# nyu-systems/Grendel-GS

Measured on AMD Instinct MI355X. Metric: training iters/sec (fwd+bwd), higher is better.
Workload: dtype f32

## Files before the change

### grendel-gs_amd/csrc/loss.hip

```cpp
#include "common.h"

namespace {

__constant__ const float WIN[11] = {1.0283801239e-03f, 7.5987582095e-03f, 3.6000773311e-02f, 1.0936068743e-01f,
                                    2.1300552785e-01f, 2.6601171494e-01f, 2.1300552785e-01f, 1.0936068743e-01f,
                                    3.6000773311e-02f, 7.5987582095e-03f, 1.0283801239e-03f};
constexpr int LT = 512;
constexpr int VO = 1024 / LT;
constexpr int TW = 32, TH = 32;
constexpr int HW = TW + 10, HH = TH + 10;
constexpr int HSTR = TW + 8;
constexpr int TS = TW;
constexpr float SSIM_C1 = 0.01f * 0.01f;
constexpr float SSIM_C2 = 0.03f * 0.03f;

__device__ __forceinline__ float block_sum(float v, float *smem) {
    const int lane = threadIdx.x & 63, wave = threadIdx.x >> 6;
#pragma unroll
    for (int d = 32; d >= 1; d >>= 1) v += __shfl_xor(v, d, 64);
    if (lane == 0) smem[wave] = v;
    __syncthreads();
    float r = 0.f;
    for (int w = 0; w < LT / 64; w++) r += smem[w];
    __syncthreads();
    return r;
}

typedef float v2f __attribute__((ext_vector_type(2)));

__device__ __forceinline__ int loss_tile(int gxT, int gyT, int &c, int &ox, int &oy, int nwg) {
    const int lin = gsr_xcd_span_of_block(blockIdx.x, nwg);
    c = lin / (gxT * gyT);
    const int rem = lin - c * (gxT * gyT);
    const int by = rem / gxT;
    ox = (rem - by * gxT) * TW;
    oy = by * TH;
    return lin;
}
__device__ __forceinline__ bool loss_band(const int *__restrict__ band, int rows_cap, int W, int gxT, int &rows, int &gyT,
                                          int &nwg, long long &row_off) {
    nwg = gridDim.x;
    row_off = 0;
    if (!band) return true;
    const int channels = nwg / (gxT * gyT);
    const int y0 = band[0], y1 = band[1];
    rows = max(0, min(y1 - y0, rows_cap));
    gyT = (rows + TH - 1) / TH;
    nwg = channels * gxT * gyT;
    row_off = (long long)y0 * W;
    return (int)blockIdx.x < nwg;
}
constexpr int HV = (TW + 16) / 4;
static_assert(HH * HV <= LT, "one halo vector per thread");

__device__ __forceinline__ float expo_apply(const float *e, float x0, float x1, float x2) {
    return fmaf(e[0], x0, fmaf(e[1], x1, fmaf(e[2], x2, e[3])));
}

template <bool VEC, bool EXPO>
__global__ void __launch_bounds__(LT)
l1_ssim_forward_kernel(int rows, int W, int gxT, int gyT, const float *__restrict__ image, long long img_cstride,
                       const uint8_t *__restrict__ gt, float *__restrict__ partials, float *__restrict__ M1,
                       float *__restrict__ M2, float *__restrict__ M3, const int *__restrict__ band,
                       const float *__restrict__ expo) {
    __shared__ v2f sXY[HH][HW + 1];
    __shared__ v2f hAB[HH][HSTR];
    __shared__ v2f hCD[HH][HSTR];
    __shared__ float hE[HH][HSTR];
    __shared__ float red[LT / 64];
#ifndef GSR_ABL_LOSS_TWO_REDUCTIONS
    __shared__ float red2[LT / 64];
#endif
    int c, ox, oy, nwg;
    long long row_off;
    const int rows_cap = rows;
    if (!loss_band(band, rows_cap, W, gxT, rows, gyT, nwg, row_off)) {
        if (threadIdx.x < 2) partials[2 * (size_t)blockIdx.x + threadIdx.x] = 0.f;
        return;
    }
    const int tile_id = loss_tile(gxT, gyT, c, ox, oy, nwg);
    const int tid = threadIdx.x;
    const float *img_c = image + (long long)c * img_cstride + row_off;
    const uint8_t *gt_c = gt + (size_t)c * rows_cap * W;
    float e[4] = {0.f, 0.f, 0.f, 0.f};
    if (EXPO) {
#pragma unroll
        for (int i = 0; i < 4; i++) e[i] = expo[4 * c + i];
    }
    const float *img_0 = image + row_off;
    if (VEC) {
        if (tid < HH * HV) {
            const int ly = tid / HV, q = tid - ly * HV;
            const int gy = oy + ly - 5, gx0 = ox - 8 + 4 * q;
            float4 x = make_float4(0.f, 0.f, 0.f, 0.f);
            uchar4 y = make_uchar4(0, 0, 0, 0);
            if (gy >= 0 && gy < rows && gx0 >= 0 && gx0 < W) {
                if (EXPO) {
                    const float *p = img_0 + (size_t)gy * W + gx0;
                    const float4 x0 = *reinterpret_cast<const float4 *>(p);
                    const float4 x1 = *reinterpret_cast<const float4 *>(p + img_cstride);
                    const float4 x2 = *reinterpret_cast<const float4 *>(p + 2 * img_cstride);
                    x = make_float4(expo_apply(e, x0.x, x1.x, x2.x), expo_apply(e, x0.y, x1.y, x2.y),
                                    expo_apply(e, x0.z, x1.z, x2.z), expo_apply(e, x0.w, x1.w, x2.w));
                } else {
                    x = *reinterpret_cast<const float4 *>(img_c + (size_t)gy * W + gx0);
                }
                y = *reinterpret_cast<const uchar4 *>(gt_c + (size_t)gy * W + gx0);
            }
            const float xs[4] = {x.x, x.y, x.z, x.w};
            const float ys[4] = {(float)y.x, (float)y.y, (float)y.z, (float)y.w};
#pragma unroll
            for (int i = 0; i < 4; i++) {
                const int lx = 4 * q - 3 + i;
                if (lx >= 0 && lx < HW) sXY[ly][lx] = v2f{xs[i], ys[i] * (1.0f / 255.0f)};
            }
        }
    } else {
        for (int idx = tid; idx < HH * HW; idx += LT) {
            const int ly = idx / HW, lx = idx % HW;
            const int gy = oy + ly - 5, gx = ox + lx - 5;
            v2f v = {0.f, 0.f};
            if (gy >= 0 && gy < rows && gx >= 0 && gx < W) {
                if (EXPO) {
                    const float *p = img_0 + (size_t)gy * W + gx;
                    v.x = expo_apply(e, p[0], p[img_cstride], p[2 * img_cstride]);
                } else {
                    v.x = img_c[(size_t)gy * W + gx];
                }
                v.y = (float)gt_c[(size_t)gy * W + gx] * (1.0f / 255.0f);
            }
            sXY[ly][lx] = v;
        }
    }
    __syncthreads();
    for (int task = tid; task < HH * (TW / 4); task += LT) {
        const int r = task / (TW / 4), cx0 = (task % (TW / 4)) * 4;
        v2f xy[14], sq[14];
        float pr[14];
#pragma unroll
        for (int i = 0; i < 14; i++) {
            xy[i] = sXY[r][cx0 + i];
            sq[i] = xy[i] * xy[i];
            pr[i] = xy[i].x * xy[i].y;
#ifndef GSR_ABL_LOSS_FWD_OUTPUT_PAIRS
            asm("" : "+v"(pr[i]));
#endif
        }
#pragma unroll
        for (int o = 0; o < 4; o++) {
            v2f a = {0.f, 0.f}, b = {0.f, 0.f};
            float e = 0.f;
#pragma unroll
            for (int k = 0; k < 11; k++) {
                const float w = WIN[k];
                a += xy[o + k] * w;
                b += sq[o + k] * w;
                e += pr[o + k] * w;
            }
            hAB[r][cx0 + o] = a;
            hCD[r][cx0 + o] = b;
            hE[r][cx0 + o] = e;
        }
    }
    __syncthreads();
    const int tx = tid % TW, ty0 = (tid / TW) * VO;
    v2f vab[VO], vcd[VO];
    float ve[VO];
    {
        v2f p[10 + VO], q[10 + VO];
        float t[10 + VO];
#pragma unroll
        for (int i = 0; i < 10 + VO; i++) {
            p[i] = hAB[ty0 + i][tx];
            q[i] = hCD[ty0 + i][tx];
            t[i] = hE[ty0 + i][tx];
#ifndef GSR_ABL_LOSS_FWD_OUTPUT_PAIRS
            asm("" : "+v"(t[i]));
#endif
        }
#pragma unroll
        for (int o = 0; o < VO; o++) {
            v2f a = {0.f, 0.f}, b = {0.f, 0.f};
            float e = 0.f;
#pragma unroll
            for (int k = 0; k < 11; k++) {
                const float w = WIN[k];
                a += p[o + k] * w;
                b += q[o + k] * w;
                e += t[o + k] * w;
            }
            vab[o] = a;
            vcd[o] = b;
            ve[o] = e;
        }
    }
    const int gx = ox + tx;
    float l1 = 0.f, ssim_sum = 0.f;
#pragma unroll
    for (int o = 0; o < VO; o++) {
        const int ty = ty0 + o, gy = oy + ty;
        if (gy < rows && gx < W) {
            const float mu1 = vab[o].x, mu2 = vab[o].y, e11 = vcd[o].x, e22 = vcd[o].y, e12 = ve[o];
            const v2f cxy = sXY[ty + 5][tx + 5];
            const float x = cxy.x, y = cxy.y;
            const float mu1_sq = mu1 * mu1, mu2_sq = mu2 * mu2, mu12 = mu1 * mu2;
            const float s1 = e11 - mu1_sq, s2 = e22 - mu2_sq, s12 = e12 - mu12;
            const float A = 2.f * mu12 + SSIM_C1, B = 2.f * s12 + SSIM_C2;
            const float Cd = mu1_sq + mu2_sq + SSIM_C1, Dd = s1 + s2 + SSIM_C2;
            const float inv_d = __builtin_amdgcn_rcpf(Dd);
            const float inv = __builtin_amdgcn_rcpf(Cd) * inv_d;
            const float ssim = A * B * inv;
            ssim_sum += ssim;
            l1 += fabsf(x - y);
            if (M1) {
                const size_t off = ((size_t)c * rows_cap + gy) * W + gx;
                M1[off] = 2.f * mu2 * (B - A) * inv - ssim * 2.f * mu1 * (Dd - Cd) * inv;
                M2[off] = -ssim * inv_d;
                M3[off] = 2.f * A * inv;
            }
        }
    }
#ifdef GSR_ABL_LOSS_TWO_REDUCTIONS
    const float sl1 = block_sum(l1, red);
    const float sss = block_sum(ssim_sum, red);
#else
    float sl1 = l1, sss = ssim_sum;
#pragma unroll
    for (int d = 32; d >= 1; d >>= 1) sl1 += __shfl_xor(sl1, d, 64);
#pragma unroll
    for (int d = 32; d >= 1; d >>= 1) sss += __shfl_xor(sss, d, 64);
    if ((tid & 63) == 0) {
        red[tid >> 6] = sl1;
        red2[tid >> 6] = sss;
    }
    __syncthreads();
    sl1 = sss = 0.f;
    for (int w = 0; w < LT / 64; w++) sl1 += red[w];
    for (int w = 0; w < LT / 64; w++) sss += red2[w];
#endif
    if (tid == 0) {
        partials[2 * (size_t)tile_id] = sl1;
        partials[2 * (size_t)tile_id + 1] = sss;
    }
}

template <bool VEC>
__global__ void __launch_bounds__(LT)
l1_ssim_backward_kernel(int rows, int W, int gxT, int gyT, const float *__restrict__ image, long long img_cstride,
                        const uint8_t *__restrict__ gt, const float *__restrict__ M1, const float *__restrict__ M2,
                        const float *__restrict__ M3, const float *__restrict__ grad_l1_sum,
                        const float *__restrict__ grad_ssim_sum, float scale_l1, float scale_ssim,
                        float *__restrict__ grad_image, long long grad_cstride, const int *__restrict__ band) {
    __shared__ float sM[3][HH][HW + 1];
    __shared__ float hor[3][HH][HSTR];
    int c, ox, oy, nwg;
    long long row_off;
    const int rows_cap = rows;
    if (!loss_band(band, rows_cap, W, gxT, rows, gyT, nwg, row_off)) return;
    loss_tile(gxT, gyT, c, ox, oy, nwg);
    const int tid = threadIdx.x;
    const size_t cbase = (size_t)c * rows_cap * W;
    if (VEC) {
        if (tid < HH * HV) {
            const int ly = tid / HV, q = tid - ly * HV;
            const int gy = oy + ly - 5, gx0 = ox - 8 + 4 * q;
            float4 a = make_float4(0.f, 0.f, 0.f, 0.f), b = a, d = a;
            if (gy >= 0 && gy < rows && gx0 >= 0 && gx0 < W) {
                const size_t o = cbase + (size_t)gy * W + gx0;
                a = *reinterpret_cast<const float4 *>(M1 + o);
                b = *reinterpret_cast<const float4 *>(M2 + o);
                d = *reinterpret_cast<const float4 *>(M3 + o);
            }
            const float as[4] = {a.x, a.y, a.z, a.w}, bs[4] = {b.x, b.y, b.z, b.w}, ds[4] = {d.x, d.y, d.z, d.w};
#pragma unroll
            for (int i = 0; i < 4; i++) {
                const int lx = 4 * q - 3 + i;
                if (lx >= 0 && lx < HW) {
                    sM[0][ly][lx] = as[i];
                    sM[1][ly][lx] = bs[i];
                    sM[2][ly][lx] = ds[i];
                }
            }
        }
    } else {
        for (int idx = tid; idx < HH * HW; idx += LT) {
            const int ly = idx / HW, lx = idx % HW;
            const int gy = oy + ly - 5, gx = ox + lx - 5;
            float a = 0.f, b = 0.f, d = 0.f;
            if (gy >= 0 && gy < rows && gx >= 0 && gx < W) {
                const size_t o = cbase + (size_t)gy * W + gx;
                a = M1[o];
                b = M2[o];
                d = M3[o];
            }
            sM[0][ly][lx] = a;
            sM[1][ly][lx] = b;
            sM[2][ly][lx] = d;
        }
    }
    __syncthreads();
    for (int task = tid; task < HH * (TW / 4); task += LT) {
        const int r = task / (TW / 4), cx0 = (task % (TW / 4)) * 4;
#pragma unroll
        for (int m = 0; m < 3; m++) {
            float v[14];
#pragma unroll
            for (int i = 0; i < 14; i++) v[i] = sM[m][r][cx0 + i];
#pragma unroll
            for (int o = 0; o < 4; o++) {
                float a = 0.f;
#pragma unroll
                for (int k = 0; k < 11; k++) a += WIN[k] * v[o + k];
                hor[m][r][cx0 + o] = a;
            }
        }
    }
    __syncthreads();
    const int tx = tid % TW, ty0 = (tid / TW) * VO;
    float cv[3][VO];
#pragma unroll
    for (int m = 0; m < 3; m++) {
        float v[10 + VO];
#pragma unroll
        for (int i = 0; i < 10 + VO; i++) v[i] = hor[m][ty0 + i][tx];
#pragma unroll
        for (int o = 0; o < VO; o++) {
            float a = 0.f;
#pragma unroll
            for (int k = 0; k < 11; k++) a += WIN[k] * v[o + k];
            cv[m][o] = a;
        }
    }
    const int gx = ox + tx;
    if (gx >= W) return;
    const float gl1 = grad_l1_sum[0] * scale_l1, gss = grad_ssim_sum[0] * scale_ssim;
#pragma unroll
    for (int o = 0; o < VO; o++) {
        const int gy = oy + ty0 + o;
        if (gy >= rows) break;
        const float x = image[(long long)c * img_cstride + row_off + (size_t)gy * W + gx];
        const float y = (float)gt[cbase + (size_t)gy * W + gx] * (1.0f / 255.0f);
        const float d = x - y;
        const float sgn = (d > 0.f ? 1.f : 0.f) - (d < 0.f ? 1.f : 0.f);
        grad_image[(long long)c * grad_cstride + row_off + (size_t)gy * W + gx] =
            gl1 * sgn + gss * (cv[0][o] + 2.f * x * cv[1][o] + y * cv[2][o]);
    }
}

__global__ void __launch_bounds__(256) l1_ssim_finalize_kernel(int nb, const float *__restrict__ partials, float c_l1,
                                                                float c_ssim, float bias, float inv_n,
                                                                float *__restrict__ out) {
    __shared__ double red[2][4];
    double a = 0.0, b = 0.0;
    const float2 *p2 = reinterpret_cast<const float2 *>(partials);
    for (int i0 = threadIdx.x; i0 < nb; i0 += 256 * 8) {
        float2 v[8];
#pragma unroll
        for (int u = 0; u < 8; u++) v[u] = p2[min(i0 + 256 * u, nb - 1)];
#pragma unroll
        for (int u = 0; u < 8; u++)
            if (i0 + 256 * u < nb) {
                a += (double)v[u].x;
                b += (double)v[u].y;
            }
    }
#pragma unroll
    for (int d = 32; d >= 1; d >>= 1) {
        a += __shfl_xor(a, d, 64);
        b += __shfl_xor(b, d, 64);
    }
    if ((threadIdx.x & 63) == 0) {
        red[0][threadIdx.x >> 6] = a;
        red[1][threadIdx.x >> 6] = b;
    }
    __syncthreads();
    if (threadIdx.x == 0) {
        const float s1 = (float)(red[0][0] + red[0][1] + red[0][2] + red[0][3]);
        const float s2 = (float)(red[1][0] + red[1][1] + red[1][2] + red[1][3]);
        out[0] = c_l1 * s1 + c_ssim * s2 + bias;
        out[1] = s1 * inv_n;
        out[2] = s2 * inv_n;
    }
}

template <bool VEC>
__global__ void __launch_bounds__(LT)
l1_ssim_backward_exposure_kernel(int rows, int W, int gxT, int gyT, const float *__restrict__ image, long long img_cstride,
                                 const uint8_t *__restrict__ gt, const float *__restrict__ M1,
                                 const float *__restrict__ M2, const float *__restrict__ M3,
                                 const float *__restrict__ grad_l1_sum, const float *__restrict__ grad_ssim_sum,
                                 float scale_l1, float scale_ssim, float *__restrict__ grad_image, long long grad_cstride,
                                 const int *__restrict__ band, const float *__restrict__ expo,
                                 float *__restrict__ expo_partials) {
    __shared__ float sM[3][HH][HW + 1];
    __shared__ float hor[3][HH][HSTR];
    __shared__ float red[12][LT / 64];
    int c0, ox, oy, nwg;
    long long row_off;
    const int rows_cap = rows;
    if (!loss_band(band, rows_cap, W, gxT, rows, gyT, nwg, row_off)) {
        if (threadIdx.x < 12) expo_partials[12 * (size_t)blockIdx.x + threadIdx.x] = 0.f;
        return;
    }
    const int tile_id = loss_tile(gxT, gyT, c0, ox, oy, nwg);
    const int tid = threadIdx.x, lane = tid & 63, wave = tid >> 6;
    const int tx = tid % TW, ty0 = (tid / TW) * VO;
    const int gx = ox + tx;
    const float gl1 = grad_l1_sum[0] * scale_l1, gss = grad_ssim_sum[0] * scale_ssim;
    float xin[3][VO], gout[3][VO];
    bool ok[VO];
#pragma unroll
    for (int o = 0; o < VO; o++) {
        const int gy = oy + ty0 + o;
        ok[o] = gx < W && gy < rows;
#pragma unroll
        for (int k = 0; k < 3; k++) {
            xin[k][o] = ok[o] ? image[(long long)k * img_cstride + row_off + (size_t)gy * W + gx] : 0.f;
            gout[k][o] = 0.f;
        }
    }
#pragma unroll 1
    for (int c = 0; c < 3; c++) {
        const size_t cbase = (size_t)c * rows_cap * W;
        if (VEC) {
            if (tid < HH * HV) {
                const int ly = tid / HV, q = tid - ly * HV;
                const int gy = oy + ly - 5, gx0 = ox - 8 + 4 * q;
                float4 a = make_float4(0.f, 0.f, 0.f, 0.f), b = a, d = a;
                if (gy >= 0 && gy < rows && gx0 >= 0 && gx0 < W) {
                    const size_t o = cbase + (size_t)gy * W + gx0;
                    a = *reinterpret_cast<const float4 *>(M1 + o);
                    b = *reinterpret_cast<const float4 *>(M2 + o);
                    d = *reinterpret_cast<const float4 *>(M3 + o);
                }
                const float as[4] = {a.x, a.y, a.z, a.w}, bs[4] = {b.x, b.y, b.z, b.w}, ds[4] = {d.x, d.y, d.z, d.w};
#pragma unroll
                for (int i = 0; i < 4; i++) {
                    const int lx = 4 * q - 3 + i;
                    if (lx >= 0 && lx < HW) {
                        sM[0][ly][lx] = as[i];
                        sM[1][ly][lx] = bs[i];
                        sM[2][ly][lx] = ds[i];
                    }
                }
            }
        } else {
            for (int idx = tid; idx < HH * HW; idx += LT) {
                const int ly = idx / HW, lx = idx % HW;
                const int gy = oy + ly - 5, gxh = ox + lx - 5;
                float a = 0.f, b = 0.f, d = 0.f;
                if (gy >= 0 && gy < rows && gxh >= 0 && gxh < W) {
                    const size_t o = cbase + (size_t)gy * W + gxh;
                    a = M1[o];
                    b = M2[o];
                    d = M3[o];
                }
                sM[0][ly][lx] = a;
                sM[1][ly][lx] = b;
                sM[2][ly][lx] = d;
            }
        }
        __syncthreads();
        for (int task = tid; task < HH * (TW / 4); task += LT) {
            const int r = task / (TW / 4), cx0 = (task % (TW / 4)) * 4;
#pragma unroll
            for (int m = 0; m < 3; m++) {
                float v[14];
#pragma unroll
                for (int i = 0; i < 14; i++) v[i] = sM[m][r][cx0 + i];
#pragma unroll
                for (int o = 0; o < 4; o++) {
                    float a = 0.f;
#pragma unroll
                    for (int k = 0; k < 11; k++) a = fmaf(WIN[k], v[o + k], a);
                    hor[m][r][cx0 + o] = a;
                }
            }
        }
        __syncthreads();
        float cv[3][VO];
#pragma unroll
        for (int m = 0; m < 3; m++) {
            float v[10 + VO];
#pragma unroll
            for (int i = 0; i < 10 + VO; i++) v[i] = hor[m][ty0 + i][tx];
#pragma unroll
            for (int o = 0; o < VO; o++) {
                float a = 0.f;
#pragma unroll
                for (int k = 0; k < 11; k++) a = fmaf(WIN[k], v[o + k], a);
                cv[m][o] = a;
            }
        }
        float e[4];
#pragma unroll
        for (int i = 0; i < 4; i++) e[i] = expo[4 * c + i];
        float s[4] = {0.f, 0.f, 0.f, 0.f};
#pragma unroll
        for (int o = 0; o < VO; o++) {
            float gp = 0.f;
            if (ok[o]) {
                const int gy = oy + ty0 + o;
                const float x = expo_apply(e, xin[0][o], xin[1][o], xin[2][o]);
                const float y = (float)gt[cbase + (size_t)gy * W + gx] * (1.0f / 255.0f);
                const float d = x - y;
                const float sgn = (d > 0.f ? 1.f : 0.f) - (d < 0.f ? 1.f : 0.f);
                const float inner = __fadd_rn(__fadd_rn(cv[0][o], __fmul_rn(__fmul_rn(2.f, x), cv[1][o])),
                                              __fmul_rn(y, cv[2][o]));
                gp = __fadd_rn(__fmul_rn(gl1, sgn), __fmul_rn(gss, inner));
            }
#pragma unroll
            for (int k = 0; k < 3; k++) {
                gout[k][o] = fmaf(e[k], gp, gout[k][o]);
                s[k] = fmaf(gp, xin[k][o], s[k]);
            }
            s[3] += gp;
        }
#pragma unroll
        for (int j = 0; j < 4; j++) {
            float v = s[j];
#pragma unroll
            for (int d = 32; d >= 1; d >>= 1) v += __shfl_xor(v, d, 64);
            if (lane == 0) red[4 * c + j][wave] = v;
        }
    }
    __syncthreads();
    if (tid < 12) {
        float r = 0.f;
        for (int w = 0; w < LT / 64; w++) r += red[tid][w];
        expo_partials[12 * (size_t)tile_id + tid] = r;
    }
#pragma unroll
    for (int o = 0; o < VO; o++) {
        if (!ok[o]) continue;
        const int gy = oy + ty0 + o;
#pragma unroll
        for (int k = 0; k < 3; k++)
            grad_image[(long long)k * grad_cstride + row_off + (size_t)gy * W + gx] = gout[k][o];
    }
}

constexpr int EXPO_GROUPS = 21;
__global__ void __launch_bounds__(256) exposure_finalize_kernel(int nrows, const float *__restrict__ partials,
                                                                 float *__restrict__ out12) {
    __shared__ double red[EXPO_GROUPS][12];
    const int t = threadIdx.x;
    if (t < 12 * EXPO_GROUPS) {
        const long long n = 12LL * nrows;
        double a = 0.0;
        for (long long i0 = t; i0 < n; i0 += 12 * EXPO_GROUPS * 8) {
            float v[8];
#pragma unroll
            for (int u = 0; u < 8; u++) v[u] = partials[min(i0 + 12 * EXPO_GROUPS * u, n - 1)];
#pragma unroll
            for (int u = 0; u < 8; u++)
                if (i0 + 12 * EXPO_GROUPS * u < n) a += (double)v[u];
        }
        red[t / 12][t % 12] = a;
    }
    __syncthreads();
    if (t < 12) {
        double r = 0.0;
        for (int g = 0; g < EXPO_GROUPS; g++) r += red[g][t];
        out12[t] = (float)r;
    }
}

}

static inline bool aligned_to(const void *p, uintptr_t a) { return (reinterpret_cast<uintptr_t>(p) & (a - 1)) == 0; }

extern "C" int gsr_l1_ssim_num_partials(int channels, int rows, int width) {
    if (channels <= 0 || rows <= 0 || width <= 0) return 0;
    return channels * gsr_div_up(rows, TS) * gsr_div_up(width, TS);
}

static int l1_ssim_forward_impl(int channels, int rows, int width, const float *image, int64_t image_channel_stride,
                                const uint8_t *gt, float *partials, float *dm_dmu1, float *dm_dE11, float *dm_dE12,
                                const int *band, const float *expo, gsr_stream_t stream) {
    if (channels <= 0 || rows < 0 || width <= 0) return GSR_EINVAL;
    if (rows == 0) return 0;
    if (!image || !gt || !partials) return GSR_EINVAL;
    if ((dm_dmu1 || dm_dE11 || dm_dE12) && !(dm_dmu1 && dm_dE11 && dm_dE12)) return GSR_EINVAL;
    const int gxT = gsr_div_up(width, TS), gyT = gsr_div_up(rows, TS);
    const dim3 grid(gxT * gyT * channels);
    const bool vec = width % 4 == 0 && image_channel_stride % 4 == 0 && aligned_to(image, 16) && aligned_to(gt, 4);
    auto kernel = expo ? (vec ? l1_ssim_forward_kernel<true, true> : l1_ssim_forward_kernel<false, true>)
                       : (vec ? l1_ssim_forward_kernel<true, false> : l1_ssim_forward_kernel<false, false>);
    hipLaunchKernelGGL(kernel, grid, dim3(LT), 0, reinterpret_cast<hipStream_t>(stream), rows, width, gxT, gyT, image,
                       (long long)image_channel_stride, gt, partials, dm_dmu1, dm_dE11, dm_dE12, band, expo);
    GSR_LAUNCH_CHECK();
    return 0;
}

extern "C" int gsr_l1_ssim_forward(int channels, int rows, int width, const float *image, int64_t image_channel_stride,
                                   const uint8_t *gt, float *partials, float *dm_dmu1, float *dm_dE11,
                                   float *dm_dE12, gsr_stream_t stream) {
    return l1_ssim_forward_impl(channels, rows, width, image, image_channel_stride, gt, partials, dm_dmu1, dm_dE11,
                                dm_dE12, nullptr, nullptr, stream);
}

extern "C" int gsr_l1_ssim_forward_band(int channels, int rows_capacity, int width, const float *image,
                                        int64_t image_channel_stride, const uint8_t *gt, float *partials,
                                        float *dm_dmu1, float *dm_dE11, float *dm_dE12, const int32_t *band_rows,
                                        gsr_stream_t stream) {
    if (!band_rows || rows_capacity <= 0) return GSR_EINVAL;
    return l1_ssim_forward_impl(channels, rows_capacity, width, image, image_channel_stride, gt, partials, dm_dmu1,
                                dm_dE11, dm_dE12, band_rows, nullptr, stream);
}

static int l1_ssim_backward_impl(int channels, int rows, int width, const float *image,
                                 int64_t image_channel_stride, const uint8_t *gt, const float *dm_dmu1,
                                 const float *dm_dE11, const float *dm_dE12, const float *grad_l1_sum,
                                 const float *grad_ssim_sum, float scale_l1, float scale_ssim, float *grad_image,
                                 int64_t grad_channel_stride, const int *band, gsr_stream_t stream) {
    if (channels <= 0 || rows < 0 || width <= 0) return GSR_EINVAL;
    if (rows == 0) return 0;
    if (!image || !gt || !dm_dmu1 || !dm_dE11 || !dm_dE12 || !grad_l1_sum || !grad_ssim_sum || !grad_image)
        return GSR_EINVAL;
    const int gxT = gsr_div_up(width, TS), gyT = gsr_div_up(rows, TS);
    const dim3 grid(gxT * gyT * channels);
    const bool vec = width % 4 == 0 && aligned_to(dm_dmu1, 16) && aligned_to(dm_dE11, 16) && aligned_to(dm_dE12, 16);
    if (vec)
        hipLaunchKernelGGL(l1_ssim_backward_kernel<true>, grid, dim3(LT), 0, reinterpret_cast<hipStream_t>(stream), rows,
                           width, gxT, gyT, image, (long long)image_channel_stride, gt, dm_dmu1, dm_dE11, dm_dE12,
                           grad_l1_sum, grad_ssim_sum, scale_l1, scale_ssim, grad_image, (long long)grad_channel_stride,
                           band);
    else
        hipLaunchKernelGGL(l1_ssim_backward_kernel<false>, grid, dim3(LT), 0, reinterpret_cast<hipStream_t>(stream), rows,
                           width, gxT, gyT, image, (long long)image_channel_stride, gt, dm_dmu1, dm_dE11, dm_dE12,
                           grad_l1_sum, grad_ssim_sum, scale_l1, scale_ssim, grad_image, (long long)grad_channel_stride,
                           band);
    GSR_LAUNCH_CHECK();
    return 0;
}

extern "C" int gsr_l1_ssim_backward(int channels, int rows, int width, const float *image,
                                    int64_t image_channel_stride, const uint8_t *gt, const float *dm_dmu1,
                                    const float *dm_dE11, const float *dm_dE12, const float *grad_l1_sum,
                                    const float *grad_ssim_sum, float scale_l1, float scale_ssim, float *grad_image,
                                    int64_t grad_channel_stride, gsr_stream_t stream) {
    return l1_ssim_backward_impl(channels, rows, width, image, image_channel_stride, gt, dm_dmu1, dm_dE11, dm_dE12,
                                 grad_l1_sum, grad_ssim_sum, scale_l1, scale_ssim, grad_image, grad_channel_stride,
                                 nullptr, stream);
}

extern "C" int gsr_l1_ssim_backward_band(int channels, int rows_capacity, int width, const float *image,
                                         int64_t image_channel_stride, const uint8_t *gt, const float *dm_dmu1,
                                         const float *dm_dE11, const float *dm_dE12, const float *grad_l1_sum,
                                         const float *grad_ssim_sum, float scale_l1, float scale_ssim,
                                         float *grad_image, int64_t grad_channel_stride, const int32_t *band_rows,
                                         gsr_stream_t stream) {
    if (!band_rows || rows_capacity <= 0) return GSR_EINVAL;
    return l1_ssim_backward_impl(channels, rows_capacity, width, image, image_channel_stride, gt, dm_dmu1, dm_dE11,
                                 dm_dE12, grad_l1_sum, grad_ssim_sum, scale_l1, scale_ssim, grad_image,
                                 grad_channel_stride, band_rows, stream);
}

extern "C" int gsr_l1_ssim_finalize(int num_partials, const float *partials, float c_l1, float c_ssim, float bias,
                                    float inv_n, float *out3, gsr_stream_t stream) {
    if (num_partials < 0 || !out3 || (num_partials > 0 && !partials) || !aligned_to(partials, 8)) return GSR_EINVAL;
    hipLaunchKernelGGL(l1_ssim_finalize_kernel, dim3(1), dim3(256), 0, reinterpret_cast<hipStream_t>(stream),
                       num_partials, partials, c_l1, c_ssim, bias, inv_n, out3);
    GSR_LAUNCH_CHECK();
    return 0;
}

extern "C" int gsr_l1_ssim_exposure_num_partials(int rows, int width) {
    if (rows <= 0 || width <= 0) return 0;
    return gsr_div_up(rows, TS) * gsr_div_up(width, TS);
}

extern "C" int gsr_l1_ssim_forward_exposure(int channels, int rows_capacity, int width, const float *image,
                                            int64_t image_channel_stride, const uint8_t *gt, float *partials,
                                            float *dm_dmu1, float *dm_dE11, float *dm_dE12, const int32_t *band_rows,
                                            const float *exposure, gsr_stream_t stream) {
    if (channels != 3 || !exposure) return GSR_EINVAL;
    if (band_rows && rows_capacity <= 0) return GSR_EINVAL;
    return l1_ssim_forward_impl(channels, rows_capacity, width, image, image_channel_stride, gt, partials, dm_dmu1,
                                dm_dE11, dm_dE12, band_rows, exposure, stream);
}

extern "C" int gsr_l1_ssim_backward_exposure(int channels, int rows_capacity, int width, const float *image,
                                             int64_t image_channel_stride, const uint8_t *gt, const float *dm_dmu1,
                                             const float *dm_dE11, const float *dm_dE12, const float *grad_l1_sum,
                                             const float *grad_ssim_sum, float scale_l1, float scale_ssim,
                                             float *grad_image, int64_t grad_channel_stride, const int32_t *band_rows,
                                             const float *exposure, float *exposure_partials, float *grad_exposure,
                                             gsr_stream_t stream) {
    const int rows = rows_capacity;
    if (channels != 3 || rows < 0 || width <= 0 || (band_rows && rows <= 0)) return GSR_EINVAL;
    if (!exposure || !exposure_partials || !grad_exposure) return GSR_EINVAL;
    if (!image || !gt || !dm_dmu1 || !dm_dE11 || !dm_dE12 || !grad_l1_sum || !grad_ssim_sum || !grad_image)
        return GSR_EINVAL;
    hipStream_t st = reinterpret_cast<hipStream_t>(stream);
    const int gxT = gsr_div_up(width, TS), gyT = gsr_div_up(rows, TS);
    if (rows > 0) {
        const bool vec = width % 4 == 0 && aligned_to(dm_dmu1, 16) && aligned_to(dm_dE11, 16) && aligned_to(dm_dE12, 16);
        auto kernel = vec ? l1_ssim_backward_exposure_kernel<true> : l1_ssim_backward_exposure_kernel<false>;
        hipLaunchKernelGGL(kernel, dim3(gxT * gyT), dim3(LT), 0, st, rows, width, gxT, gyT, image,
                           (long long)image_channel_stride, gt, dm_dmu1, dm_dE11, dm_dE12, grad_l1_sum, grad_ssim_sum,
                           scale_l1, scale_ssim, grad_image, (long long)grad_channel_stride, band_rows, exposure,
                           exposure_partials);
        GSR_LAUNCH_CHECK();
    }
    hipLaunchKernelGGL(exposure_finalize_kernel, dim3(1), dim3(256), 0, st, gxT * gyT, exposure_partials, grad_exposure);
    GSR_LAUNCH_CHECK();
    return 0;
}
```

Before: 835.6.

## Merge SSIM second-moment maps and shrink LDS to fit more workgroups

The forward SSIM kernel now blurs x²+y² as one sum instead of blurring x² and y² separately, since only their sum feeds the variance denominator. This cuts the intermediate maps from five to four and drops the separate hE LDS buffer. The horizontal-pass row stride is reduced for both forward and backward kernels, and launch bounds now request 8 waves per SIMD, so more workgroups can be resident per CU. Map writes use 32-bit tile-relative byte offsets, guarded by a new width limit, and fusing the squared terms before blurring may change rounding slightly.

Result: no change. 842.9 (median of 6 runs) (+0.9%).

```diff
diff --git a/grendel-gs_amd/csrc/loss.hip b/grendel-gs_amd/csrc/loss.hip
--- a/grendel-gs_amd/csrc/loss.hip
+++ b/grendel-gs_amd/csrc/loss.hip
@@ -11,6 +11,21 @@
 constexpr int HW = TW + 10, HH = TH + 10;
 constexpr int HSTR = TW + 8;
 constexpr int TS = TW;
+#if defined(GSR_ABL_LOSS_FIVE_MAPS) && !defined(GSR_ABL_LOSS_FWD_3WG)
+#define GSR_ABL_LOSS_FWD_3WG
+#endif
+#ifdef GSR_ABL_LOSS_FWD_3WG
+constexpr int HSTR_F = HSTR;
+#define LOSS_FWD_BOUNDS __launch_bounds__(LT)
+#else
+constexpr int HSTR_F = TW + 4;
+#define LOSS_FWD_BOUNDS __launch_bounds__(LT, 8)
+#endif
+#ifdef GSR_ABL_LOSS_BWD_3WG
+constexpr int HSTR_B = HSTR;
+#else
+constexpr int HSTR_B = TW + 4;
+#endif
 constexpr float SSIM_C1 = 0.01f * 0.01f;
 constexpr float SSIM_C2 = 0.03f * 0.03f;
 
@@ -58,15 +73,19 @@
 }
 
 template <bool VEC, bool EXPO>
-__global__ void __launch_bounds__(LT)
+__global__ void LOSS_FWD_BOUNDS
 l1_ssim_forward_kernel(int rows, int W, int gxT, int gyT, const float *__restrict__ image, long long img_cstride,
                        const uint8_t *__restrict__ gt, float *__restrict__ partials, float *__restrict__ M1,
                        float *__restrict__ M2, float *__restrict__ M3, const int *__restrict__ band,
                        const float *__restrict__ expo) {
     __shared__ v2f sXY[HH][HW + 1];
-    __shared__ v2f hAB[HH][HSTR];
-    __shared__ v2f hCD[HH][HSTR];
-    __shared__ float hE[HH][HSTR];
+    __shared__ v2f hAB[HH][HSTR_F];
+#ifdef GSR_ABL_LOSS_FIVE_MAPS
+    __shared__ v2f hCD[HH][HSTR_F];
+    __shared__ float hE[HH][HSTR_F];
+#else
+    __shared__ v2f hCD[HH][HSTR_F];
+#endif
     __shared__ float red[LT / 64];
 #ifndef GSR_ABL_LOSS_TWO_REDUCTIONS
     __shared__ float red2[LT / 64];
@@ -135,6 +154,26 @@
     __syncthreads();
     for (int task = tid; task < HH * (TW / 4); task += LT) {
         const int r = task / (TW / 4), cx0 = (task % (TW / 4)) * 4;
+#ifndef GSR_ABL_LOSS_FIVE_MAPS
+        v2f xy[14], sp[14];
+#pragma unroll
+        for (int i = 0; i < 14; i++) {
+            xy[i] = sXY[r][cx0 + i];
+            sp[i] = v2f{fmaf(xy[i].y, xy[i].y, xy[i].x * xy[i].x), xy[i].x * xy[i].y};
+        }
+#pragma unroll
+        for (int o = 0; o < 4; o++) {
+            v2f a = {0.f, 0.f}, b = {0.f, 0.f};
+#pragma unroll
+            for (int k = 0; k < 11; k++) {
+                const float w = WIN[k];
+                a += xy[o + k] * w;
+                b += sp[o + k] * w;
+            }
+            hAB[r][cx0 + o] = a;
+            hCD[r][cx0 + o] = b;
+        }
+#else
         v2f xy[14], sq[14];
         float pr[14];
 #pragma unroll
@@ -161,10 +200,33 @@
             hCD[r][cx0 + o] = b;
             hE[r][cx0 + o] = e;
         }
+#endif
     }
     __syncthreads();
     const int tx = tid % TW, ty0 = (tid / TW) * VO;
     v2f vab[VO], vcd[VO];
+#ifndef GSR_ABL_LOSS_FIVE_MAPS
+    {
+        v2f p[10 + VO], q[10 + VO];
+#pragma unroll
+        for (int i = 0; i < 10 + VO; i++) {
+            p[i] = hAB[ty0 + i][tx];
+            q[i] = hCD[ty0 + i][tx];
+        }
+#pragma unroll
+        for (int o = 0; o < VO; o++) {
+            v2f a = {0.f, 0.f}, b = {0.f, 0.f};
+#pragma unroll
+            for (int k = 0; k < 11; k++) {
+                const float w = WIN[k];
+                a += p[o + k] * w;
+                b += q[o + k] * w;
+            }
+            vab[o] = a;
+            vcd[o] = b;
+        }
+    }
+#else
     float ve[VO];
     {
         v2f p[10 + VO], q[10 + VO];
@@ -194,12 +256,22 @@
             ve[o] = e;
         }
     }
+#endif
     const int gx = ox + tx;
     float l1 = 0.f, ssim_sum = 0.f;
 #pragma unroll
     for (int o = 0; o < VO; o++) {
         const int ty = ty0 + o, gy = oy + ty;
         if (gy < rows && gx < W) {
+#ifndef GSR_ABL_LOSS_FIVE_MAPS
+            const float mu1 = vab[o].x, mu2 = vab[o].y, ess = vcd[o].x, e12 = vcd[o].y;
+            const v2f cxy = sXY[ty + 5][tx + 5];
+            const float x = cxy.x, y = cxy.y;
+            const float mu1_sq = mu1 * mu1, mu2_sq = mu2 * mu2, mu12 = mu1 * mu2;
+            const float s12 = e12 - mu12;
+            const float A = 2.f * mu12 + SSIM_C1, B = 2.f * s12 + SSIM_C2;
+            const float Cd = mu1_sq + mu2_sq + SSIM_C1, Dd = (ess - (mu1_sq + mu2_sq)) + SSIM_C2;
+#else
             const float mu1 = vab[o].x, mu2 = vab[o].y, e11 = vcd[o].x, e22 = vcd[o].y, e12 = ve[o];
             const v2f cxy = sXY[ty + 5][tx + 5];
             const float x = cxy.x, y = cxy.y;
@@ -207,16 +279,25 @@
             const float s1 = e11 - mu1_sq, s2 = e22 - mu2_sq, s12 = e12 - mu12;
             const float A = 2.f * mu12 + SSIM_C1, B = 2.f * s12 + SSIM_C2;
             const float Cd = mu1_sq + mu2_sq + SSIM_C1, Dd = s1 + s2 + SSIM_C2;
+#endif
             const float inv_d = __builtin_amdgcn_rcpf(Dd);
             const float inv = __builtin_amdgcn_rcpf(Cd) * inv_d;
             const float ssim = A * B * inv;
             ssim_sum += ssim;
             l1 += fabsf(x - y);
             if (M1) {
+#ifdef GSR_ABL_LOSS_FWD_3WG
                 const size_t off = ((size_t)c * rows_cap + gy) * W + gx;
-                M1[off] = 2.f * mu2 * (B - A) * inv - ssim * 2.f * mu1 * (Dd - Cd) * inv;
-                M2[off] = -ssim * inv_d;
-                M3[off] = 2.f * A * inv;
+#define LOSS_MAP_AT(M) M[off]
+#else
+                const size_t tile_off = ((size_t)c * rows_cap + oy) * W + ox;
+                const uint32_t boff = ((uint32_t)ty * (uint32_t)W + (uint32_t)tx) * 4u;
+#define LOSS_MAP_AT(M) (*reinterpret_cast<float *>(reinterpret_cast<char *>(M + tile_off) + boff))
+#endif
+                LOSS_MAP_AT(M1) = 2.f * mu2 * (B - A) * inv - ssim * 2.f * mu1 * (Dd - Cd) * inv;
+                LOSS_MAP_AT(M2) = -ssim * inv_d;
+                LOSS_MAP_AT(M3) = 2.f * A * inv;
+#undef LOSS_MAP_AT
             }
         }
     }
@@ -252,7 +333,7 @@
                         const float *__restrict__ grad_ssim_sum, float scale_l1, float scale_ssim,
                         float *__restrict__ grad_image, long long grad_cstride, const int *__restrict__ band) {
     __shared__ float sM[3][HH][HW + 1];
-    __shared__ float hor[3][HH][HSTR];
+    __shared__ float hor[3][HH][HSTR_B];
     int c, ox, oy, nwg;
     long long row_off;
     const int rows_cap = rows;
@@ -581,6 +662,7 @@
     if (channels <= 0 || rows < 0 || width <= 0) return GSR_EINVAL;
     if (rows == 0) return 0;
     if (!image || !gt || !partials) return GSR_EINVAL;
+    if (width > (1 << 24)) return GSR_EINVAL;
     if ((dm_dmu1 || dm_dE11 || dm_dE12) && !(dm_dmu1 && dm_dE11 && dm_dE12)) return GSR_EINVAL;
     const int gxT = gsr_div_up(width, TS), gyT = gsr_div_up(rows, TS);
     const dim3 grid(gxT * gyT * channels);
```
